# KTH-RPL/HiMo

Hardware: AMD Instinct MI355X
Metric: lidar_frames_per_sec_120k (higher is better)
Workload: dtype f16x2 (two-term split fp16, x = h + l with exact subnormals, on the matrix cores; float32 accumulate; ~22-bit products); 1 GPU; per-frame pipeline: pillarise 3 sweeps (512x512 grid) -> SeFlow++-style encoder/decoder + GRU head (random-init, self-specified: reference network source absent) -> per-point flow -> ego-motion removal + dt0 + flow2compDis -> comp_dis; points_per_frame=120000, sweeps_per_frame=3, parallelism=frames sharded x1, refined_output=False, batches_in_flight=3, matrix_arithmetic=f16x2, samples_per_backbone_launch=16, collectives=none (single process)

## Files before the change

### himo_amd/csrc/gruhead.hip

```cpp
#include "conv_common.h"
#include "bf16x3.h"

namespace himo {

struct GruHeadArgs {
    int64_t n;
    const int* pid; const float* offsets;
    const float* img0; const float* img1; int img_pitch;
    const float* dec; int dec_pitch;
    const float* w_off; const float* b_off;
    const unsigned short* wzr; const float* bzr;
    const unsigned short* wq; const float* bq;
    const unsigned short* w1; const float* b1;
    const float* w2; const float* b2;
    const float* xyz_t; const float* pts; int stride;
    float* flow;
    int iters;
    int img_split;
    unsigned* nonfinite;
    int w2_pitch;
};

constexpr int kGhMaxIters = 4;
struct GruHeadSave {
    float* hx;
    float* rhx;
    float* z; float* r; float* q;
    float* pre1; float* y1;
    float* res;
    int64_t rows;
};

constexpr int kGhMaxSamples = 16;
struct GruHeadSample {
    int64_t n;
    const int* pid; const float* offsets; const float* img0; const float* img1; const float* dec;
    const float* xyz_t; const float* pts; float* flow; int stride;
};
struct GruHeadBatch {
    int n_samples;
    int block_start[kGhMaxSamples + 1];
    GruHeadSample s[kGhMaxSamples];
};

constexpr int kGhRows = 64;
constexpr bool kGhLaunder = false;

template <int SLABS>
__device__ inline int a_slot(int s, int slab, int row, int half) {
    return ((s * SLABS + slab) * kGhRows + row) * 32 + ((half ^ ((row >> 4) & 1)) << 4);
}

template <int FMT, int SLABS>
__device__ inline void a_store(unsigned char* A, int row, int k, float v) {
    constexpr int kGhPlane = SLABS * kGhRows * 32;
    unsigned h, m = 0, l;
    if (FMT == 3) split3(v, h, m, l); else split2(v, h, l);
    const int slab = k >> 4, kk = k & 15;
    const int off = a_slot<SLABS>(0, slab, row, kk >> 3) + (kk & 7) * 2;
    *reinterpret_cast<unsigned short*>(A + off) = (unsigned short)h;
    if (FMT == 3) *reinterpret_cast<unsigned short*>(A + off + kGhPlane) = (unsigned short)m;
    *reinterpret_cast<unsigned short*>(A + off + (FMT - 1) * kGhPlane) = (unsigned short)l;
}

template <int RT, int NT, int FMT, int SLABS>
__device__ inline void gemm192(const unsigned char* A, const unsigned short* __restrict__ wpk, int cout, const int (&col)[NT],
                               floatx16 (&acc)[RT][NT], int rt0, int li, int lh) {
    uint4 bcur[NT][FMT], bnxt[NT][FMT];
    auto load_b = [&](int slab, uint4 (&b)[NT][FMT]) {
#pragma unroll
        for (int t = 0; t < NT; ++t)
#pragma unroll
            for (int s = 0; s < FMT; ++s)
                b[t][s] = *reinterpret_cast<const uint4*>(wpk + (((int64_t)slab * FMT + s) * cout + col[t] + li) * 16 + lh * 8);
    };
    load_b(0, bcur);
    constexpr int kUnroll = SLABS % 2 == 0 ? 2 : 3;
#pragma unroll kUnroll
    for (int slab = 0; slab < SLABS; ++slab) {
        if (slab + 1 < SLABS) load_b(slab + 1, bnxt);
        bf16x8 af[RT][FMT];
#pragma unroll
        for (int rt = 0; rt < RT; ++rt)
#pragma unroll
            for (int s = 0; s < FMT; ++s)
                af[rt][s] = *reinterpret_cast<const bf16x8*>(A + a_slot<SLABS>(s, slab, (rt0 + rt) * 32 + li, lh));
#define HIMO_TERM(SA, SB)                                                                                          \
    _Pragma("unroll") for (int rt = 0; rt < RT; ++rt) _Pragma("unroll") for (int t = 0; t < NT; ++t)                  \
        acc[rt][t] = __builtin_amdgcn_mfma_f32_32x32x16_bf16(af[rt][SA], __builtin_bit_cast(bf16x8, bcur[t][SB]), acc[rt][t], 0, 0, 0);
#define HIMO_TERM16(ACC, SA, SB)                                                                                   \
    _Pragma("unroll") for (int rt = 0; rt < RT; ++rt) _Pragma("unroll") for (int t = 0; t < NT; ++t)                  \
        ACC[rt][t] = __builtin_amdgcn_mfma_f32_32x32x16_f16(__builtin_bit_cast(f16x8, af[rt][SA]),                    \
                                                           __builtin_bit_cast(f16x8, bcur[t][SB]), ACC[rt][t], 0, 0, 0);
        if constexpr (FMT == 3) {
            HIMO_TERM(2, 0) HIMO_TERM(0, 2) HIMO_TERM(1, 1) HIMO_TERM(1, 0) HIMO_TERM(0, 1) HIMO_TERM(0, 0)
        } else {
            HIMO_TERM16(acc, 1, 0) HIMO_TERM16(acc, 0, 1) HIMO_TERM16(acc, 0, 0)
        }
#undef HIMO_TERM16
#undef HIMO_TERM
#pragma unroll
        for (int t = 0; t < NT; ++t)
#pragma unroll
            for (int s = 0; s < FMT; ++s) bcur[t][s] = bnxt[t][s];
    }
    if (FMT == 2) {
#pragma unroll
        for (int rt = 0; rt < RT; ++rt)
#pragma unroll
            for (int t = 0; t < NT; ++t)
#pragma unroll
                for (int r = 0; r < 16; ++r)
                    acc[rt][t][r] = acc[rt][t][r] * kF16AccScale;
    }
}

template <int GROUP>
__device__ inline void sv_store(float* base, unsigned byte_off, float v) {
    *reinterpret_cast<float*>(reinterpret_cast<char*>(base) + byte_off) = v;
}

template <int FMT, int SLABS, bool SAVE = false>
__global__ __launch_bounds__(256, (FMT == 2 && !SAVE) ? 3 : 2) void gru_head_kernel(GruHeadArgs a, GruHeadBatch batch, GruHeadSave sv) {
    constexpr bool FOLD = SLABS == 9;
    static_assert(!(SAVE && FOLD), "the training forward keeps x explicit");
    constexpr int kGhPlane = SLABS * kGhRows * 32;
    __shared__ __attribute__((aligned(16))) unsigned char A[FMT * kGhPlane];
    __shared__ int s_pid[kGhRows];
    const int wave = __builtin_amdgcn_readfirstlane(threadIdx.x >> 6), lane = threadIdx.x & 63;
    const int li = lane & 31, lh = lane >> 5;
    int bid = blockIdx.x;
    {
        int smp = 0;
        while (smp + 1 < batch.n_samples && bid >= batch.block_start[smp + 1]) ++smp;
        bid -= batch.block_start[smp];
        const GruHeadSample& g = batch.s[smp];
        a.n = g.n; a.pid = g.pid; a.offsets = g.offsets; a.img0 = g.img0; a.img1 = g.img1; a.dec = g.dec;
        a.xyz_t = g.xyz_t; a.pts = g.pts; a.flow = g.flow; a.stride = g.stride;
    }
    const int64_t r0 = (int64_t)bid * kGhRows;

    if (threadIdx.x < kGhRows) {
        const int64_t i = r0 + threadIdx.x;
        s_pid[threadIdx.x] = i < a.n ? a.pid[i] : -1;
    }
    if constexpr (FOLD) {
        const int row = threadIdx.x >> 2, q = threadIdx.x & 3;
        const int64_t i = r0 + row;
        float v[4] = {0.f, 0.f, 0.f, 0.f};
        if (q == 0) {
            if (i < a.n) { v[0] = a.offsets[i * 3]; v[1] = a.offsets[i * 3 + 1]; v[2] = a.offsets[i * 3 + 2]; }
            v[3] = 1.f;
        }
#pragma unroll
        for (int k = 0; k < 4; ++k) a_store<FMT, SLABS>(A, row, 128 + q * 4 + k, v[k]);
    } else if constexpr (SAVE) {
        const int c = threadIdx.x & 63;
        const float w0 = a.w_off[c], w1 = a.w_off[64 + c], w2 = a.w_off[128 + c], bc = a.b_off[c];
#pragma unroll 4
        for (int j = 0; j < 16; ++j) {
            const int row = wave + 4 * j;
            const int64_t i = r0 + row;
            const int64_t ic = i < a.n ? i : a.n - 1;
            const float o0 = a.offsets[ic * 3], o1 = a.offsets[ic * 3 + 1], o2 = a.offsets[ic * 3 + 2];
            const float v = fmaf(o2, w2, fmaf(o1, w1, o0 * w0)) + bc;
            a_store<FMT, SLABS>(A, row, 128 + c, v);
            const unsigned at = ((unsigned)i * 192u + 128u + (unsigned)c) * 4u;
            for (int t = 0; t <= a.iters; ++t) sv_store<0>(sv.hx + t * sv.rows * 192, at, v);
            for (int t = 0; t < a.iters; ++t) sv_store<0>(sv.rhx + t * sv.rows * 192, at, v);
        }
    } else {
        const int row = threadIdx.x >> 2, q = threadIdx.x & 3;
        const int64_t i = r0 + row;
        float o0 = 0.f, o1 = 0.f, o2 = 0.f;
        if (i < a.n) { o0 = a.offsets[i * 3]; o1 = a.offsets[i * 3 + 1]; o2 = a.offsets[i * 3 + 2]; }
#pragma unroll
        for (int k = 0; k < 16; ++k) {
            const int c = q * 16 + k;
            const float v = fmaf(o2, a.w_off[128 + c], fmaf(o1, a.w_off[64 + c], o0 * a.w_off[c])) + a.b_off[c];
            a_store<FMT, SLABS>(A, row, 128 + c, v);
        }
    }
    __syncthreads();

    const float* src = wave == 0 ? a.img0 : wave == 1 ? a.img1 : a.dec + (wave - 2) * 32;
    const int src_pitch = wave < 2 ? a.img_pitch : a.dec_pitch;
    float h[2][16];
    {
        int cell[2][16];
#pragma unroll
        for (int rt = 0; rt < 2; ++rt)
#pragma unroll
            for (int r = 0; r < 16; ++r) cell[rt][r] = s_pid[rt * 32 + (r & 3) + 8 * (r >> 2) + 4 * lh];
        if (FMT == 2 && wave < 2 && a.img_split) {
            unsigned short hh[2][16], ll[2][16];
#pragma unroll
            for (int rt = 0; rt < 2; ++rt)
#pragma unroll
                for (int r = 0; r < 16; ++r) {
                    const unsigned short* rec = reinterpret_cast<const unsigned short*>(src + (int64_t)max(cell[rt][r], 0) * src_pitch + (li & ~15));
                    hh[rt][r] = rec[li & 15]; ll[rt][r] = rec[16 + (li & 15)];
                }
#pragma unroll
            for (int rt = 0; rt < 2; ++rt)
#pragma unroll
                for (int r = 0; r < 16; ++r)
                    h[rt][r] = cell[rt][r] >= 0 ? (float)__builtin_bit_cast(_Float16, hh[rt][r]) + (float)__builtin_bit_cast(_Float16, ll[rt][r]) : 0.f;
        } else {
#pragma unroll
            for (int rt = 0; rt < 2; ++rt)
#pragma unroll
                for (int r = 0; r < 16; ++r) h[rt][r] = src[(int64_t)max(cell[rt][r], 0) * src_pitch + li];
#pragma unroll
            for (int rt = 0; rt < 2; ++rt)
#pragma unroll
                for (int r = 0; r < 16; ++r) h[rt][r] = cell[rt][r] >= 0 ? h[rt][r] : 0.f;
            if (FMT == 2 && wave < 2) {
#pragma unroll
                for (int rt = 0; rt < 2; ++rt)
#pragma unroll
                    for (int r = 0; r < 16; ++r) {
                        unsigned hh, ll;
                        split2(h[rt][r], hh, ll);
                        h[rt][r] = (float)__builtin_bit_cast(_Float16, (unsigned short)hh) + (float)__builtin_bit_cast(_Float16, (unsigned short)ll);
                    }
            }
        }
#pragma unroll
        for (int rt = 0; rt < 2; ++rt)
#pragma unroll
            for (int r = 0; r < 16; ++r) {
                const int row = rt * 32 + (r & 3) + 8 * (r >> 2) + 4 * lh;
                a_store<FMT, SLABS>(A, row, wave * 32 + li, h[rt][r]);
                if constexpr (SAVE) sv_store<1>(sv.hx, (((unsigned)r0 + row) * 192u + wave * 32 + li) * 4u, h[rt][r]);
            }
    }
    __syncthreads();
    unsigned o128 = (((unsigned)r0 + 4 * lh) * 128u + wave * 32 + li) * 4u, o192 = (((unsigned)r0 + 4 * lh) * 192u + wave * 32 + li) * 4u;

    const int col_zr[2] = {wave * 32, 128 + wave * 32};
    const int col_q[1] = {wave * 32};
    const float bz = a.bzr[wave * 32 + li], br = a.bzr[128 + wave * 32 + li], bq = a.bq[wave * 32 + li];

#pragma unroll 1
    for (int it = 0; it < a.iters; ++it) {
        int sli = li, slh = lh;
        if constexpr (SAVE || kGhLaunder) asm volatile("" : "+v"(o128), "+v"(o192), "+v"(sli), "+v"(slh));
        float* const sz = SAVE ? sv.z + it * sv.rows * 128 : nullptr; float* const sr = SAVE ? sv.r + it * sv.rows * 128 : nullptr;
        float* const sq = SAVE ? sv.q + it * sv.rows * 128 : nullptr; float* const srhx = SAVE ? sv.rhx + it * sv.rows * 192 : nullptr;
        float* const shx = SAVE ? sv.hx + (it + 1) * sv.rows * 192 : nullptr;
        floatx16 acc[2][2];
#pragma unroll
        for (int rt = 0; rt < 2; ++rt)
#pragma unroll
            for (int t = 0; t < 2; ++t)
#pragma unroll
                for (int r = 0; r < 16; ++r) acc[rt][t][r] = 0.f;
        gemm192<2, 2, FMT, SLABS>(A, a.wzr, 256, col_zr, acc, 0, li, lh);
        __syncthreads();
#pragma unroll
        for (int rt = 0; rt < 2; ++rt)
#pragma unroll
            for (int r = 0; r < 16; ++r) {
                acc[rt][0][r] = sigmoid_f(acc[rt][0][r] + bz);
                const float rr = sigmoid_f(acc[rt][1][r] + br);
                const int row = rt * 32 + (r & 3) + 8 * (r >> 2) + 4 * slh;
                a_store<FMT, SLABS>(A, row, wave * 32 + sli, rr * h[rt][r]);
                if constexpr (SAVE) {
                    const unsigned dr = rt * 32 + (r & 3) + 8 * (r >> 2);
                    sv_store<2>(sz, o128 + dr * 512u, acc[rt][0][r]); sv_store<2>(sr, o128 + dr * 512u, rr);
                    sv_store<3>(srhx, o192 + dr * 768u, rr * h[rt][r]);
                }
            }
        __syncthreads();
        if constexpr (SAVE || kGhLaunder) asm volatile("" : "+v"(o128), "+v"(o192), "+v"(sli), "+v"(slh));
        floatx16 acq[2][1];
#pragma unroll
        for (int rt = 0; rt < 2; ++rt)
#pragma unroll
            for (int r = 0; r < 16; ++r) acq[rt][0][r] = 0.f;
        gemm192<2, 1, FMT, SLABS>(A, a.wq, 128, col_q, acq, 0, li, lh);
        __syncthreads();
#pragma unroll
        for (int rt = 0; rt < 2; ++rt)
#pragma unroll
            for (int r = 0; r < 16; ++r) {
                const float q = tanh_f(acq[rt][0][r] + bq);
                const float zz = acc[rt][0][r];
                const float hn = (1.0f - zz) * h[rt][r] + zz * q;
                h[rt][r] = hn;
                const int row = rt * 32 + (r & 3) + 8 * (r >> 2) + 4 * slh;
                a_store<FMT, SLABS>(A, row, wave * 32 + sli, hn);
                if constexpr (SAVE) {
                    const unsigned dr = rt * 32 + (r & 3) + 8 * (r >> 2);
                    sv_store<4>(sq, o128 + dr * 512u, q);
                    sv_store<5>(shx, o192 + dr * 768u, hn);
                }
            }
        __syncthreads();
    }

    floatx16 ac1[1][1];
#pragma unroll
    for (int r = 0; r < 16; ++r) ac1[0][0][r] = 0.f;
    const int col_1[1] = {0};
    if (wave < 2) gemm192<1, 1, FMT, SLABS>(A, a.w1, 32, col_1, ac1, wave, li, lh);
    __syncthreads();
    float* Y = reinterpret_cast<float*>(A);
    if (wave < 2) {
        const float b1 = a.b1[li];
#pragma unroll
        for (int r = 0; r < 16; ++r) {
            const int row = wave * 32 + (r & 3) + 8 * (r >> 2) + 4 * lh;
            const float pre = ac1[0][0][r] + b1, y = gelu_exact(pre);
            Y[row * 32 + li] = y;
            if constexpr (SAVE) {
                const unsigned at = (((unsigned)r0 + row) * 32u + li) * 4u;
                sv_store<6>(sv.pre1, at, pre); sv_store<6>(sv.y1, at, y);
            }
        }
    }
    __syncthreads();
    if constexpr (SAVE) {
        const int row = threadIdx.x >> 2, c = threadIdx.x & 3;
        const int64_t i = r0 + row;
        float out = 0.f;
        if (c < 3 && s_pid[row] >= 0) {
            const float* y = Y + row * 32;
            float s = y[0] * a.w2[c];
#pragma unroll
            for (int k = 1; k < 32; ++k) s = fmaf(y[k], a.w2[k * a.w2_pitch + c], s);
            out = s + a.b2[c];
        }
        sv.res[i * 4 + c] = out;
        if (a.nonfinite && !(fabsf(out) <= 3.4028234664e38f)) atomicOr(a.nonfinite, 1u);
        return;
    }
    if (threadIdx.x < 3 * kGhRows) {
        const int row = threadIdx.x / 3, c = threadIdx.x % 3;
        const int64_t i = r0 + row;
        if (i < a.n) {
            const float pose_flow = a.xyz_t[i * 3 + c] - a.pts[i * a.stride + c];
            float out = pose_flow;
            if (s_pid[row] >= 0) {
                const float* y = Y + row * 32;
                float s = y[0] * a.w2[c];
#pragma unroll
                for (int k = 1; k < 32; ++k) s = fmaf(y[k], a.w2[k * a.w2_pitch + c], s);
                out = pose_flow + (s + a.b2[c]);
            }
            a.flow[i * 3 + c] = out;
            if (a.nonfinite && !(fabsf(out) <= 3.4028234664e38f)) atomicOr(a.nonfinite, 1u);
        }
    }
}

}

using namespace himo;

static int gru_head_launch(int n_samples, const himo_head_sample* h_samples, int img_pitch, int dec_pitch,
                           const float* d_w_off, const float* d_b_off, bool folded,
                           const void* d_wzr_packed, const float* d_bzr, const void* d_wq_packed, const float* d_bq,
                           const void* d_w1_packed, const float* d_b1, const float* d_w2, const float* d_b2,
                           int iters, int packed_format, int img_split, unsigned* d_nonfinite, void* stream) {
    if (img_split && (packed_format != 1 || (img_pitch & 15))) return HIMO_ERR_INVALID_ARGUMENT;
    if (n_samples < 0 || n_samples > kGhMaxSamples || (n_samples && !h_samples)) return HIMO_ERR_INVALID_ARGUMENT;
    if (iters < 0 || !(packed_format == 0 || packed_format == 1) || img_pitch < 32 || dec_pitch < 64) return HIMO_ERR_INVALID_ARGUMENT;
    if ((!folded && (!d_w_off || !d_b_off)) || !d_wzr_packed || !d_bzr || !d_wq_packed || !d_bq || !d_w1_packed || !d_b1 || !d_w2 || !d_b2)
        return HIMO_ERR_INVALID_ARGUMENT;
    if ((reinterpret_cast<uintptr_t>(d_wzr_packed) | reinterpret_cast<uintptr_t>(d_wq_packed) | reinterpret_cast<uintptr_t>(d_w1_packed)) & 15)
        return HIMO_ERR_INVALID_ARGUMENT;
    GruHeadBatch b{};
    int64_t blocks = 0;
    for (int i = 0; i < n_samples; ++i) {
        const himo_head_sample& h = h_samples[i];
        if (h.n < 0 || h.pc_stride < 3) return HIMO_ERR_INVALID_ARGUMENT;
        if (h.n == 0) continue;
        if (!h.d_pid || !h.d_offsets || !h.d_img0 || !h.d_img1 || !h.d_dec || !h.d_xyz_t || !h.d_pts || !h.d_flow) return HIMO_ERR_INVALID_ARGUMENT;
        GruHeadSample& g = b.s[b.n_samples];
        g.n = h.n; g.pid = h.d_pid; g.offsets = h.d_offsets; g.img0 = h.d_img0; g.img1 = h.d_img1; g.dec = h.d_dec;
        g.xyz_t = h.d_xyz_t; g.pts = h.d_pts; g.flow = h.d_flow; g.stride = h.pc_stride;
        b.block_start[b.n_samples] = (int)blocks;
        blocks += (h.n + kGhRows - 1) / kGhRows;
        if (blocks > 0x7fffffff) return HIMO_ERR_INVALID_ARGUMENT;
        b.block_start[++b.n_samples] = (int)blocks;
    }
    if (!blocks) return HIMO_OK;
    GruHeadArgs a{};
    a.img_pitch = img_pitch; a.dec_pitch = dec_pitch; a.w_off = d_w_off; a.b_off = d_b_off;
    a.wzr = (const unsigned short*)d_wzr_packed; a.bzr = d_bzr; a.wq = (const unsigned short*)d_wq_packed; a.bq = d_bq;
    a.w1 = (const unsigned short*)d_w1_packed; a.b1 = d_b1; a.w2 = d_w2; a.b2 = d_b2; a.iters = iters;
    a.img_split = img_split ? 1 : 0;
    a.nonfinite = d_nonfinite;
    a.w2_pitch = 3;
    hipStream_t s = (hipStream_t)stream;
    ProfScope ps("gru_head_kernel", s);
    const dim3 grid((unsigned)blocks);
    const GruHeadSave none{};
    if (folded) {
        if (packed_format == 1) hipLaunchKernelGGL((gru_head_kernel<2, 9>), grid, dim3(256), 0, s, a, b, none);
        else hipLaunchKernelGGL((gru_head_kernel<3, 9>), grid, dim3(256), 0, s, a, b, none);
    } else {
        if (packed_format == 1) hipLaunchKernelGGL((gru_head_kernel<2, 12>), grid, dim3(256), 0, s, a, b, none);
        else hipLaunchKernelGGL((gru_head_kernel<3, 12>), grid, dim3(256), 0, s, a, b, none);
    }
    HIMO_LAUNCH_CHECK("gru_head_kernel");
    return HIMO_OK;
}

extern "C" int himo_gru_head_batch(int n_samples, const himo_head_sample* h_samples, int img_pitch, int dec_pitch,
                                   const float* d_w_off, const float* d_b_off,
                                   const void* d_wzr_packed, const float* d_bzr, const void* d_wq_packed, const float* d_bq,
                                   const void* d_w1_packed, const float* d_b1, const float* d_w2, const float* d_b2,
                                   int iters, int packed_format, int img_split, void* stream) {
    return gru_head_launch(n_samples, h_samples, img_pitch, dec_pitch, d_w_off, d_b_off, false, d_wzr_packed, d_bzr, d_wq_packed, d_bq,
                           d_w1_packed, d_b1, d_w2, d_b2, iters, packed_format, img_split, nullptr, stream);
}

extern "C" int himo_gru_head_batch_folded(int n_samples, const himo_head_sample* h_samples, int img_pitch, int dec_pitch,
                                          const void* d_wzr_packed, const float* d_bzr, const void* d_wq_packed, const float* d_bq,
                                          const void* d_w1_packed, const float* d_b1, const float* d_w2, const float* d_b2,
                                          int iters, int packed_format, int img_split, void* stream) {
    return gru_head_launch(n_samples, h_samples, img_pitch, dec_pitch, nullptr, nullptr, true, d_wzr_packed, d_bzr, d_wq_packed, d_bq,
                           d_w1_packed, d_b1, d_w2, d_b2, iters, packed_format, img_split, nullptr, stream);
}

extern "C" int himo_gru_head_batch_guarded(int n_samples, const himo_head_sample* h_samples, int img_pitch, int dec_pitch,
                                           const float* d_w_off, const float* d_b_off,
                                           const void* d_wzr_packed, const float* d_bzr, const void* d_wq_packed, const float* d_bq,
                                           const void* d_w1_packed, const float* d_b1, const float* d_w2, const float* d_b2,
                                           int iters, int packed_format, int img_split, uint32_t* d_nonfinite, void* stream) {
    if ((d_w_off == nullptr) != (d_b_off == nullptr)) return HIMO_ERR_INVALID_ARGUMENT;
    return gru_head_launch(n_samples, h_samples, img_pitch, dec_pitch, d_w_off, d_b_off, d_w_off == nullptr, d_wzr_packed, d_bzr, d_wq_packed,
                           d_bq, d_w1_packed, d_b1, d_w2, d_b2, iters, packed_format, img_split, d_nonfinite, stream);
}

extern "C" int himo_gru_head_train(int64_t n, const int32_t* d_pid, const float* d_offsets, const float* d_img0, const float* d_img1,
                                   int img_pitch, const float* d_dec, int dec_pitch, const float* d_w_off, const float* d_b_off,
                                   const void* d_wzr_packed, const float* d_bzr, const void* d_wq_packed, const float* d_bq,
                                   const void* d_w1_packed, const float* d_b1, const float* d_w2, int w2_pitch, const float* d_b2,
                                   int iters, int packed_format, const himo_head_saved* h_saved, uint32_t* d_nonfinite, void* stream) {
    if (n < 0 || iters < 1 || iters > kGhMaxIters || !(packed_format == 0 || packed_format == 1) || img_pitch < 32 || dec_pitch < 64 ||
        !(w2_pitch == 3 || w2_pitch == 4) || !h_saved)
        return HIMO_ERR_INVALID_ARGUMENT;
    if (!d_w_off || !d_b_off || !d_wzr_packed || !d_bzr || !d_wq_packed || !d_bq || !d_w1_packed || !d_b1 || !d_w2 || !d_b2)
        return HIMO_ERR_INVALID_ARGUMENT;
    if ((reinterpret_cast<uintptr_t>(d_wzr_packed) | reinterpret_cast<uintptr_t>(d_wq_packed) | reinterpret_cast<uintptr_t>(d_w1_packed)) & 15)
        return HIMO_ERR_INVALID_ARGUMENT;
    if (n == 0) return HIMO_OK;
    if (!d_pid || !d_offsets || !d_img0 || !d_img1 || !d_dec) return HIMO_ERR_INVALID_ARGUMENT;
    if (h_saved && h_saved->rows * 768 >= ((int64_t)1 << 32)) return HIMO_ERR_UNSUPPORTED;
    GruHeadSave sv{};
    sv.hx = h_saved->d_hx; sv.rhx = h_saved->d_rhx; sv.z = h_saved->d_z; sv.r = h_saved->d_r; sv.q = h_saved->d_q;
    sv.pre1 = h_saved->d_pre1; sv.y1 = h_saved->d_y1; sv.res = h_saved->d_res;
    sv.rows = h_saved->rows;
    if (!sv.hx || !sv.rhx || !sv.z || !sv.r || !sv.q || !sv.pre1 || !sv.y1 || !sv.res || sv.rows < (n + 63) / 64 * 64 || (sv.rows & 63))
        return HIMO_ERR_INVALID_ARGUMENT;
    GruHeadBatch b{};
    b.n_samples = 1;
    GruHeadSample& g = b.s[0];
    g.n = n; g.pid = d_pid; g.offsets = d_offsets; g.img0 = d_img0; g.img1 = d_img1; g.dec = d_dec;
    const int64_t blocks = (n + kGhRows - 1) / kGhRows;
    if (blocks > 0x7fffffff) return HIMO_ERR_INVALID_ARGUMENT;
    b.block_start[0] = 0; b.block_start[1] = (int)blocks;
    GruHeadArgs a{};
    a.img_pitch = img_pitch; a.dec_pitch = dec_pitch; a.w_off = d_w_off; a.b_off = d_b_off;
    a.wzr = (const unsigned short*)d_wzr_packed; a.bzr = d_bzr; a.wq = (const unsigned short*)d_wq_packed; a.bq = d_bq;
    a.w1 = (const unsigned short*)d_w1_packed; a.b1 = d_b1; a.w2 = d_w2; a.b2 = d_b2; a.iters = iters; a.w2_pitch = w2_pitch;
    a.nonfinite = d_nonfinite;
    hipStream_t s = (hipStream_t)stream;
    ProfScope ps("gru_head_train_kernel", s);
    if (packed_format == 1) hipLaunchKernelGGL((gru_head_kernel<2, 12, true>), dim3((unsigned)blocks), dim3(256), 0, s, a, b, sv);
    else hipLaunchKernelGGL((gru_head_kernel<3, 12, true>), dim3((unsigned)blocks), dim3(256), 0, s, a, b, sv);
    HIMO_LAUNCH_CHECK("gru_head_kernel<train>");
    return HIMO_OK;
}

extern "C" int himo_clear_u32(uint32_t* d_words, int n, void* stream) {
    if (!d_words || n < 1) return HIMO_ERR_INVALID_ARGUMENT;
    HIMO_HIP(hipMemsetAsync(d_words, 0, (size_t)n * 4, (hipStream_t)stream));
    return HIMO_OK;
}

extern "C" int himo_gru_head(int64_t n, const int32_t* d_pid, const float* d_offsets, const float* d_img0, const float* d_img1,
                             int img_pitch, const float* d_dec, int dec_pitch, const float* d_w_off, const float* d_b_off,
                             const void* d_wzr_packed, const float* d_bzr, const void* d_wq_packed, const float* d_bq,
                             const void* d_w1_packed, const float* d_b1, const float* d_w2, const float* d_b2,
                             const float* d_xyz_t, const float* d_pts, int pc_stride, float* d_flow, int iters, int packed_format,
                             void* stream) {
    himo_head_sample h{n, d_pid, d_offsets, d_img0, d_img1, d_dec, d_xyz_t, d_pts, pc_stride, d_flow};
    return himo_gru_head_batch(1, &h, img_pitch, dec_pitch, d_w_off, d_b_off, d_wzr_packed, d_bzr, d_wq_packed, d_bq,
                               d_w1_packed, d_b1, d_w2, d_b2, iters, packed_format, 0, stream);
}
```

Baseline: 757.6 frames/s.

## Widen folded f16x2 GRU head blocks to 128 rows with buffer-load double-buffered weights

The folded f16x2 GRU head now processes 128 rows per 256-thread block, so each wave handles four row tiles and every weight fragment loaded from global memory feeds twice as many MFMAs. The weight loads switch to raw buffer loads through a buffer resource, and the slab loop is restructured into an explicit two-buffer ping-pong that computes one row tile at a time. Separately, the r*h product and the GRU blend are computed with contraction disabled, and the product is split into two fp16 terms via an fma residual. The trade-off is twice the LDS per block and a lower occupancy target (2 blocks instead of 3), plus higher register pressure from the larger accumulator arrays.

```diff
diff --git a/himo_amd/csrc/gruhead.hip b/himo_amd/csrc/gruhead.hip
--- a/himo_amd/csrc/gruhead.hip
+++ b/himo_amd/csrc/gruhead.hip
@@ -44,65 +44,104 @@
 };
 
 constexpr int kGhRows = 64;
+constexpr int kGhRowsWide = 128;
 constexpr bool kGhLaunder = false;
 
-template <int SLABS>
+template <int SLABS, int ROWS>
 __device__ inline int a_slot(int s, int slab, int row, int half) {
-    return ((s * SLABS + slab) * kGhRows + row) * 32 + ((half ^ ((row >> 4) & 1)) << 4);
-}
-
-template <int FMT, int SLABS>
+    return ((s * SLABS + slab) * ROWS + row) * 32 + ((half ^ ((row >> 4) & 1)) << 4);
+}
+
+template <int FMT, int SLABS, int ROWS>
 __device__ inline void a_store(unsigned char* A, int row, int k, float v) {
-    constexpr int kGhPlane = SLABS * kGhRows * 32;
+    constexpr int kGhPlane = SLABS * ROWS * 32;
     unsigned h, m = 0, l;
     if (FMT == 3) split3(v, h, m, l); else split2(v, h, l);
     const int slab = k >> 4, kk = k & 15;
-    const int off = a_slot<SLABS>(0, slab, row, kk >> 3) + (kk & 7) * 2;
+    const int off = a_slot<SLABS, ROWS>(0, slab, row, kk >> 3) + (kk & 7) * 2;
     *reinterpret_cast<unsigned short*>(A + off) = (unsigned short)h;
     if (FMT == 3) *reinterpret_cast<unsigned short*>(A + off + kGhPlane) = (unsigned short)m;
     *reinterpret_cast<unsigned short*>(A + off + (FMT - 1) * kGhPlane) = (unsigned short)l;
 }
 
-template <int RT, int NT, int FMT, int SLABS>
+template <int FMT, int SLABS, int ROWS>
+__device__ inline void a_store_prod(unsigned char* A, int row, int k, float r, float h) {
+    if constexpr (FMT == 2) {
+#pragma clang fp contract(off)
+        const _Float16 hh = (_Float16)(r * h);
+        const _Float16 ll = (_Float16)fmaf(r, h, -(float)hh);
+        const int slab = k >> 4, kk = k & 15;
+        const int off = a_slot<SLABS, ROWS>(0, slab, row, kk >> 3) + (kk & 7) * 2;
+        *reinterpret_cast<unsigned short*>(A + off) = __builtin_bit_cast(unsigned short, hh);
+        *reinterpret_cast<unsigned short*>(A + off + SLABS * ROWS * 32) = __builtin_bit_cast(unsigned short, ll);
+    } else {
+        a_store<FMT, SLABS, ROWS>(A, row, k, r * h);
+    }
+}
+template <int FMT>
+__device__ inline float gru_blend(float z, float h, float q) {
+    if constexpr (FMT == 2) {
+#pragma clang fp contract(off)
+        const float a = (1.0f - z) * h, b = z * q;
+        return a + b;
+    } else {
+        return (1.0f - z) * h + z * q;
+    }
+}
+
+template <int RT, int NT, int FMT, int SLABS, int ROWS>
 __device__ inline void gemm192(const unsigned char* A, const unsigned short* __restrict__ wpk, int cout, const int (&col)[NT],
                                floatx16 (&acc)[RT][NT], int rt0, int li, int lh) {
-    uint4 bcur[NT][FMT], bnxt[NT][FMT];
+    uint4 b0[NT][FMT], b1[NT][FMT];
+    const __amdgpu_buffer_rsrc_t wrsrc = __builtin_amdgcn_make_buffer_rsrc(const_cast<unsigned short*>(wpk), 0, SLABS * FMT * cout * 32, 0x00020000);
+    const int lane_off = li * 32 + lh * 16;
     auto load_b = [&](int slab, uint4 (&b)[NT][FMT]) {
+        typedef unsigned u32x4 __attribute__((ext_vector_type(4)));
 #pragma unroll
         for (int t = 0; t < NT; ++t)
 #pragma unroll
+            for (int s = 0; s < FMT; ++s) {
+                const u32x4 v = __builtin_amdgcn_raw_buffer_load_b128(wrsrc, lane_off, ((slab * FMT + s) * cout + col[t]) * 32, 0);
+                b[t][s] = __builtin_bit_cast(uint4, v);
+            }
+    };
+    auto step = [&](int slab, const uint4 (&b)[NT][FMT]) {
+#pragma unroll
+        for (int rt = 0; rt < RT; ++rt) {
+            bf16x8 af[FMT];
+#pragma unroll
             for (int s = 0; s < FMT; ++s)
-                b[t][s] = *reinterpret_cast<const uint4*>(wpk + (((int64_t)slab * FMT + s) * cout + col[t] + li) * 16 + lh * 8);
-    };
-    load_b(0, bcur);
-    constexpr int kUnroll = SLABS % 2 == 0 ? 2 : 3;
-#pragma unroll kUnroll
-    for (int slab = 0; slab < SLABS; ++slab) {
-        if (slab + 1 < SLABS) load_b(slab + 1, bnxt);
-        bf16x8 af[RT][FMT];
-#pragma unroll
-        for (int rt = 0; rt < RT; ++rt)
-#pragma unroll
-            for (int s = 0; s < FMT; ++s)
-                af[rt][s] = *reinterpret_cast<const bf16x8*>(A + a_slot<SLABS>(s, slab, (rt0 + rt) * 32 + li, lh));
+                af[s] = *reinterpret_cast<const bf16x8*>(A + a_slot<SLABS, ROWS>(s, slab, (rt0 + rt) * 32 + li, lh));
 #define HIMO_TERM(SA, SB)                                                                                          \
-    _Pragma("unroll") for (int rt = 0; rt < RT; ++rt) _Pragma("unroll") for (int t = 0; t < NT; ++t)                  \
-        acc[rt][t] = __builtin_amdgcn_mfma_f32_32x32x16_bf16(af[rt][SA], __builtin_bit_cast(bf16x8, bcur[t][SB]), acc[rt][t], 0, 0, 0);
-#define HIMO_TERM16(ACC, SA, SB)                                                                                   \
-    _Pragma("unroll") for (int rt = 0; rt < RT; ++rt) _Pragma("unroll") for (int t = 0; t < NT; ++t)                  \
-        ACC[rt][t] = __builtin_amdgcn_mfma_f32_32x32x16_f16(__builtin_bit_cast(f16x8, af[rt][SA]),                    \
-                                                           __builtin_bit_cast(f16x8, bcur[t][SB]), ACC[rt][t], 0, 0, 0);
-        if constexpr (FMT == 3) {
-            HIMO_TERM(2, 0) HIMO_TERM(0, 2) HIMO_TERM(1, 1) HIMO_TERM(1, 0) HIMO_TERM(0, 1) HIMO_TERM(0, 0)
-        } else {
-            HIMO_TERM16(acc, 1, 0) HIMO_TERM16(acc, 0, 1) HIMO_TERM16(acc, 0, 0)
-        }
+    _Pragma("unroll") for (int t = 0; t < NT; ++t)                                                                    \
+        acc[rt][t] = __builtin_amdgcn_mfma_f32_32x32x16_bf16(af[SA], __builtin_bit_cast(bf16x8, b[t][SB]), acc[rt][t], 0, 0, 0);
+#define HIMO_TERM16(SA, SB)                                                                                        \
+    _Pragma("unroll") for (int t = 0; t < NT; ++t)                                                                    \
+        acc[rt][t] = __builtin_amdgcn_mfma_f32_32x32x16_f16(__builtin_bit_cast(f16x8, af[SA]),                        \
+                                                           __builtin_bit_cast(f16x8, b[t][SB]), acc[rt][t], 0, 0, 0);
+            if constexpr (FMT == 3) {
+                HIMO_TERM(2, 0) HIMO_TERM(0, 2) HIMO_TERM(1, 1) HIMO_TERM(1, 0) HIMO_TERM(0, 1) HIMO_TERM(0, 0)
+            } else {
+                HIMO_TERM16(1, 0) HIMO_TERM16(0, 1) HIMO_TERM16(0, 0)
+            }
 #undef HIMO_TERM16
 #undef HIMO_TERM
-#pragma unroll
-        for (int t = 0; t < NT; ++t)
-#pragma unroll
-            for (int s = 0; s < FMT; ++s) bcur[t][s] = bnxt[t][s];
+        }
+    };
+    load_b(0, b0);
+#pragma unroll 1
+    for (int slab = 0; slab + 2 < SLABS; slab += 2) {
+        load_b(slab + 1, b1);
+        step(slab, b0);
+        load_b(slab + 2, b0);
+        step(slab + 1, b1);
+    }
+    if constexpr (SLABS % 2 == 1) {
+        step(SLABS - 1, b0);
+    } else {
+        load_b(SLABS - 1, b1);
+        step(SLABS - 2, b0);
+        step(SLABS - 1, b1);
     }
     if (FMT == 2) {
 #pragma unroll
@@ -120,13 +159,16 @@
     *reinterpret_cast<float*>(reinterpret_cast<char*>(base) + byte_off) = v;
 }
 
-template <int FMT, int SLABS, bool SAVE = false>
-__global__ __launch_bounds__(256, (FMT == 2 && !SAVE) ? 3 : 2) void gru_head_kernel(GruHeadArgs a, GruHeadBatch batch, GruHeadSave sv) {
+template <int FMT, int SLABS, bool SAVE = false, int ROWS = kGhRows>
+__global__ __launch_bounds__(256, (FMT == 2 && !SAVE && ROWS == 64) ? 3 : 2) void gru_head_kernel(GruHeadArgs a, GruHeadBatch batch, GruHeadSave sv) {
     constexpr bool FOLD = SLABS == 9;
+    constexpr int RT = ROWS / 32;
     static_assert(!(SAVE && FOLD), "the training forward keeps x explicit");
-    constexpr int kGhPlane = SLABS * kGhRows * 32;
+    static_assert(ROWS == 64 || ROWS == 128, "a wave owns 32 hidden columns of 2 or 4 row tiles");
+    static_assert(!SAVE || ROWS == kGhRows, "the saved tensors are laid out for 64-row blocks");
+    constexpr int kGhPlane = SLABS * ROWS * 32;
     __shared__ __attribute__((aligned(16))) unsigned char A[FMT * kGhPlane];
-    __shared__ int s_pid[kGhRows];
+    __shared__ int s_pid[ROWS];
     const int wave = __builtin_amdgcn_readfirstlane(threadIdx.x >> 6), lane = threadIdx.x & 63;
     const int li = lane & 31, lh = lane >> 5;
     int bid = blockIdx.x;
@@ -138,22 +180,25 @@
         a.n = g.n; a.pid = g.pid; a.offsets = g.offsets; a.img0 = g.img0; a.img1 = g.img1; a.dec = g.dec;
         a.xyz_t = g.xyz_t; a.pts = g.pts; a.flow = g.flow; a.stride = g.stride;
     }
-    const int64_t r0 = (int64_t)bid * kGhRows;
-
-    if (threadIdx.x < kGhRows) {
+    const int64_t r0 = (int64_t)bid * ROWS;
+
+    if (threadIdx.x < ROWS) {
         const int64_t i = r0 + threadIdx.x;
         s_pid[threadIdx.x] = i < a.n ? a.pid[i] : -1;
     }
     if constexpr (FOLD) {
-        const int row = threadIdx.x >> 2, q = threadIdx.x & 3;
-        const int64_t i = r0 + row;
-        float v[4] = {0.f, 0.f, 0.f, 0.f};
-        if (q == 0) {
-            if (i < a.n) { v[0] = a.offsets[i * 3]; v[1] = a.offsets[i * 3 + 1]; v[2] = a.offsets[i * 3 + 2]; }
-            v[3] = 1.f;
-        }
-#pragma unroll
-        for (int k = 0; k < 4; ++k) a_store<FMT, SLABS>(A, row, 128 + q * 4 + k, v[k]);
+#pragma unroll
+        for (int rb = 0; rb < ROWS; rb += 64) {
+            const int row = rb + (threadIdx.x >> 2), q = threadIdx.x & 3;
+            const int64_t i = r0 + row;
+            float v[4] = {0.f, 0.f, 0.f, 0.f};
+            if (q == 0) {
+                if (i < a.n) { v[0] = a.offsets[i * 3]; v[1] = a.offsets[i * 3 + 1]; v[2] = a.offsets[i * 3 + 2]; }
+                v[3] = 1.f;
+            }
+#pragma unroll
+            for (int k = 0; k < 4; ++k) a_store<FMT, SLABS, ROWS>(A, row, 128 + q * 4 + k, v[k]);
+        }
     } else if constexpr (SAVE) {
         const int c = threadIdx.x & 63;
         const float w0 = a.w_off[c], w1 = a.w_off[64 + c], w2 = a.w_off[128 + c], bc = a.b_off[c];
@@ -164,76 +209,80 @@
             const int64_t ic = i < a.n ? i : a.n - 1;
             const float o0 = a.offsets[ic * 3], o1 = a.offsets[ic * 3 + 1], o2 = a.offsets[ic * 3 + 2];
             const float v = fmaf(o2, w2, fmaf(o1, w1, o0 * w0)) + bc;
-            a_store<FMT, SLABS>(A, row, 128 + c, v);
+            a_store<FMT, SLABS, ROWS>(A, row, 128 + c, v);
             const unsigned at = ((unsigned)i * 192u + 128u + (unsigned)c) * 4u;
             for (int t = 0; t <= a.iters; ++t) sv_store<0>(sv.hx + t * sv.rows * 192, at, v);
             for (int t = 0; t < a.iters; ++t) sv_store<0>(sv.rhx + t * sv.rows * 192, at, v);
         }
     } else {
-        const int row = threadIdx.x >> 2, q = threadIdx.x & 3;
-        const int64_t i = r0 + row;
-        float o0 = 0.f, o1 = 0.f, o2 = 0.f;
-        if (i < a.n) { o0 = a.offsets[i * 3]; o1 = a.offsets[i * 3 + 1]; o2 = a.offsets[i * 3 + 2]; }
-#pragma unroll
-        for (int k = 0; k < 16; ++k) {
-            const int c = q * 16 + k;
-            const float v = fmaf(o2, a.w_off[128 + c], fmaf(o1, a.w_off[64 + c], o0 * a.w_off[c])) + a.b_off[c];
-            a_store<FMT, SLABS>(A, row, 128 + c, v);
+#pragma unroll
+        for (int rb = 0; rb < ROWS; rb += 64) {
+            const int row = rb + (threadIdx.x >> 2), q = threadIdx.x & 3;
+            const int64_t i = r0 + row;
+            float o0 = 0.f, o1 = 0.f, o2 = 0.f;
+            if (i < a.n) { o0 = a.offsets[i * 3]; o1 = a.offsets[i * 3 + 1]; o2 = a.offsets[i * 3 + 2]; }
+#pragma unroll
+            for (int k = 0; k < 16; ++k) {
+                const int c = q * 16 + k;
+                const float v = fmaf(o2, a.w_off[128 + c], fmaf(o1, a.w_off[64 + c], o0 * a.w_off[c])) + a.b_off[c];
+                a_store<FMT, SLABS, ROWS>(A, row, 128 + c, v);
+            }
         }
     }
     __syncthreads();
 
     const float* src = wave == 0 ? a.img0 : wave == 1 ? a.img1 : a.dec + (wave - 2) * 32;
     const int src_pitch = wave < 2 ? a.img_pitch : a.dec_pitch;
-    float h[2][16];
-    {
-        int cell[2][16];
-#pragma unroll
-        for (int rt = 0; rt < 2; ++rt)
-#pragma unroll
-            for (int r = 0; r < 16; ++r) cell[rt][r] = s_pid[rt * 32 + (r & 3) + 8 * (r >> 2) + 4 * lh];
-        if (FMT == 2 && wave < 2 && a.img_split) {
-            unsigned short hh[2][16], ll[2][16];
+    float h[RT][16];
+#pragma unroll
+    for (int rp = 0; rp < RT; rp += 2) {
+            int cell[2][16];
 #pragma unroll
             for (int rt = 0; rt < 2; ++rt)
 #pragma unroll
+                for (int r = 0; r < 16; ++r) cell[rt][r] = s_pid[(rp + rt) * 32 + (r & 3) + 8 * (r >> 2) + 4 * lh];
+            if (FMT == 2 && wave < 2 && a.img_split) {
+                unsigned short hh[2][16], ll[2][16];
+#pragma unroll
+                for (int rt = 0; rt < 2; ++rt)
+#pragma unroll
+                    for (int r = 0; r < 16; ++r) {
+                        const unsigned short* rec = reinterpret_cast<const unsigned short*>(src + (int64_t)max(cell[rt][r], 0) * src_pitch + (li & ~15));
+                        hh[rt][r] = rec[li & 15]; ll[rt][r] = rec[16 + (li & 15)];
+                    }
+#pragma unroll
+                for (int rt = 0; rt < 2; ++rt)
+#pragma unroll
+                    for (int r = 0; r < 16; ++r)
+                        h[rp + rt][r] = cell[rt][r] >= 0 ? (float)__builtin_bit_cast(_Float16, hh[rt][r]) + (float)__builtin_bit_cast(_Float16, ll[rt][r]) : 0.f;
+            } else {
+#pragma unroll
+                for (int rt = 0; rt < 2; ++rt)
+#pragma unroll
+                    for (int r = 0; r < 16; ++r) h[rp + rt][r] = src[(int64_t)max(cell[rt][r], 0) * src_pitch + li];
+#pragma unroll
+                for (int rt = 0; rt < 2; ++rt)
+#pragma unroll
+                    for (int r = 0; r < 16; ++r) h[rp + rt][r] = cell[rt][r] >= 0 ? h[rp + rt][r] : 0.f;
+                if (FMT == 2 && wave < 2) {
+#pragma unroll
+                    for (int rt = 0; rt < 2; ++rt)
+#pragma unroll
+                        for (int r = 0; r < 16; ++r) {
+                            unsigned hh, ll;
+                            split2(h[rp + rt][r], hh, ll);
+                            h[rp + rt][r] = (float)__builtin_bit_cast(_Float16, (unsigned short)hh) + (float)__builtin_bit_cast(_Float16, (unsigned short)ll);
+                        }
+                }
+            }
+#pragma unroll
+            for (int rt = 0; rt < 2; ++rt)
+#pragma unroll
                 for (int r = 0; r < 16; ++r) {
-                    const unsigned short* rec = reinterpret_cast<const unsigned short*>(src + (int64_t)max(cell[rt][r], 0) * src_pitch + (li & ~15));
-                    hh[rt][r] = rec[li & 15]; ll[rt][r] = rec[16 + (li & 15)];
+                    const int row = (rp + rt) * 32 + (r & 3) + 8 * (r >> 2) + 4 * lh;
+                    a_store<FMT, SLABS, ROWS>(A, row, wave * 32 + li, h[rp + rt][r]);
+                    if constexpr (SAVE) sv_store<1>(sv.hx, (((unsigned)r0 + row) * 192u + wave * 32 + li) * 4u, h[rp + rt][r]);
                 }
-#pragma unroll
-            for (int rt = 0; rt < 2; ++rt)
-#pragma unroll
-                for (int r = 0; r < 16; ++r)
-                    h[rt][r] = cell[rt][r] >= 0 ? (float)__builtin_bit_cast(_Float16, hh[rt][r]) + (float)__builtin_bit_cast(_Float16, ll[rt][r]) : 0.f;
-        } else {
-#pragma unroll
-            for (int rt = 0; rt < 2; ++rt)
-#pragma unroll
-                for (int r = 0; r < 16; ++r) h[rt][r] = src[(int64_t)max(cell[rt][r], 0) * src_pitch + li];
-#pragma unroll
-            for (int rt = 0; rt < 2; ++rt)
-#pragma unroll
-                for (int r = 0; r < 16; ++r) h[rt][r] = cell[rt][r] >= 0 ? h[rt][r] : 0.f;
-            if (FMT == 2 && wave < 2) {
-#pragma unroll
-                for (int rt = 0; rt < 2; ++rt)
-#pragma unroll
-                    for (int r = 0; r < 16; ++r) {
-                        unsigned hh, ll;
-                        split2(h[rt][r], hh, ll);
-                        h[rt][r] = (float)__builtin_bit_cast(_Float16, (unsigned short)hh) + (float)__builtin_bit_cast(_Float16, (unsigned short)ll);
-                    }
-            }
-        }
-#pragma unroll
-        for (int rt = 0; rt < 2; ++rt)
-#pragma unroll
-            for (int r = 0; r < 16; ++r) {
-                const int row = rt * 32 + (r & 3) + 8 * (r >> 2) + 4 * lh;
-                a_store<FMT, SLABS>(A, row, wave * 32 + li, h[rt][r]);
-                if constexpr (SAVE) sv_store<1>(sv.hx, (((unsigned)r0 + row) * 192u + wave * 32 + li) * 4u, h[rt][r]);
-            }
     }
     __syncthreads();
     unsigned o128 = (((unsigned)r0 + 4 * lh) * 128u + wave * 32 + li) * 4u, o192 = (((unsigned)r0 + 4 * lh) * 192u + wave * 32 + li) * 4u;
@@ -249,23 +298,23 @@
         float* const sz = SAVE ? sv.z + it * sv.rows * 128 : nullptr; float* const sr = SAVE ? sv.r + it * sv.rows * 128 : nullptr;
         float* const sq = SAVE ? sv.q + it * sv.rows * 128 : nullptr; float* const srhx = SAVE ? sv.rhx + it * sv.rows * 192 : nullptr;
         float* const shx = SAVE ? sv.hx + (it + 1) * sv.rows * 192 : nullptr;
-        floatx16 acc[2][2];
-#pragma unroll
-        for (int rt = 0; rt < 2; ++rt)
+        floatx16 acc[RT][2];
+#pragma unroll
+        for (int rt = 0; rt < RT; ++rt)
 #pragma unroll
             for (int t = 0; t < 2; ++t)
 #pragma unroll
                 for (int r = 0; r < 16; ++r) acc[rt][t][r] = 0.f;
-        gemm192<2, 2, FMT, SLABS>(A, a.wzr, 256, col_zr, acc, 0, li, lh);
+        gemm192<RT, 2, FMT, SLABS, ROWS>(A, a.wzr, 256, col_zr, acc, 0, li, lh);
         __syncthreads();
 #pragma unroll
-        for (int rt = 0; rt < 2; ++rt)
+        for (int rt = 0; rt < RT; ++rt)
 #pragma unroll
             for (int r = 0; r < 16; ++r) {
                 acc[rt][0][r] = sigmoid_f(acc[rt][0][r] + bz);
                 const float rr = sigmoid_f(acc[rt][1][r] + br);
                 const int row = rt * 32 + (r & 3) + 8 * (r >> 2) + 4 * slh;
-                a_store<FMT, SLABS>(A, row, wave * 32 + sli, rr * h[rt][r]);
+                a_store_prod<FMT, SLABS, ROWS>(A, row, wave * 32 + sli, rr, h[rt][r]);
                 if constexpr (SAVE) {
                     const unsigned dr = rt * 32 + (r & 3) + 8 * (r >> 2);
                     sv_store<2>(sz, o128 + dr * 512u, acc[rt][0][r]); sv_store<2>(sr, o128 + dr * 512u, rr);
@@ -274,23 +323,23 @@
             }
         __syncthreads();
         if constexpr (SAVE || kGhLaunder) asm volatile("" : "+v"(o128), "+v"(o192), "+v"(sli), "+v"(slh));
-        floatx16 acq[2][1];
-#pragma unroll
-        for (int rt = 0; rt < 2; ++rt)
+        floatx16 acq[RT][1];
+#pragma unroll
+        for (int rt = 0; rt < RT; ++rt)
 #pragma unroll
             for (int r = 0; r < 16; ++r) acq[rt][0][r] = 0.f;
-        gemm192<2, 1, FMT, SLABS>(A, a.wq, 128, col_q, acq, 0, li, lh);
+        gemm192<RT, 1, FMT, SLABS, ROWS>(A, a.wq, 128, col_q, acq, 0, li, lh);
         __syncthreads();
 #pragma unroll
-        for (int rt = 0; rt < 2; ++rt)
+        for (int rt = 0; rt < RT; ++rt)
 #pragma unroll
             for (int r = 0; r < 16; ++r) {
                 const float q = tanh_f(acq[rt][0][r] + bq);
                 const float zz = acc[rt][0][r];
-                const float hn = (1.0f - zz) * h[rt][r] + zz * q;
+                const float hn = gru_blend<FMT>(zz, h[rt][r], q);
                 h[rt][r] = hn;
                 const int row = rt * 32 + (r & 3) + 8 * (r >> 2) + 4 * slh;
-                a_store<FMT, SLABS>(A, row, wave * 32 + sli, hn);
+                a_store<FMT, SLABS, ROWS>(A, row, wave * 32 + sli, hn);
                 if constexpr (SAVE) {
                     const unsigned dr = rt * 32 + (r & 3) + 8 * (r >> 2);
                     sv_store<4>(sq, o128 + dr * 512u, q);
@@ -304,10 +353,10 @@
 #pragma unroll
     for (int r = 0; r < 16; ++r) ac1[0][0][r] = 0.f;
     const int col_1[1] = {0};
-    if (wave < 2) gemm192<1, 1, FMT, SLABS>(A, a.w1, 32, col_1, ac1, wave, li, lh);
+    if (wave < RT) gemm192<1, 1, FMT, SLABS, ROWS>(A, a.w1, 32, col_1, ac1, wave, li, lh);
     __syncthreads();
     float* Y = reinterpret_cast<float*>(A);
-    if (wave < 2) {
+    if (wave < RT) {
         const float b1 = a.b1[li];
 #pragma unroll
         for (int r = 0; r < 16; ++r) {
@@ -336,8 +385,8 @@
         if (a.nonfinite && !(fabsf(out) <= 3.4028234664e38f)) atomicOr(a.nonfinite, 1u);
         return;
     }
-    if (threadIdx.x < 3 * kGhRows) {
-        const int row = threadIdx.x / 3, c = threadIdx.x % 3;
+    for (int e = threadIdx.x; e < 3 * ROWS; e += 256) {
+        const int row = e / 3, c = e % 3;
         const int64_t i = r0 + row;
         if (i < a.n) {
             const float pose_flow = a.xyz_t[i * 3 + c] - a.pts[i * a.stride + c];
@@ -371,6 +420,7 @@
         return HIMO_ERR_INVALID_ARGUMENT;
     if ((reinterpret_cast<uintptr_t>(d_wzr_packed) | reinterpret_cast<uintptr_t>(d_wq_packed) | reinterpret_cast<uintptr_t>(d_w1_packed)) & 15)
         return HIMO_ERR_INVALID_ARGUMENT;
+    const int rows = (folded && packed_format == 1) ? kGhRowsWide : kGhRows;
     GruHeadBatch b{};
     int64_t blocks = 0;
     for (int i = 0; i < n_samples; ++i) {
@@ -382,7 +432,7 @@
         g.n = h.n; g.pid = h.d_pid; g.offsets = h.d_offsets; g.img0 = h.d_img0; g.img1 = h.d_img1; g.dec = h.d_dec;
         g.xyz_t = h.d_xyz_t; g.pts = h.d_pts; g.flow = h.d_flow; g.stride = h.pc_stride;
         b.block_start[b.n_samples] = (int)blocks;
-        blocks += (h.n + kGhRows - 1) / kGhRows;
+        blocks += (h.n + rows - 1) / rows;
         if (blocks > 0x7fffffff) return HIMO_ERR_INVALID_ARGUMENT;
         b.block_start[++b.n_samples] = (int)blocks;
     }
@@ -399,7 +449,7 @@
     const dim3 grid((unsigned)blocks);
     const GruHeadSave none{};
     if (folded) {
-        if (packed_format == 1) hipLaunchKernelGGL((gru_head_kernel<2, 9>), grid, dim3(256), 0, s, a, b, none);
+        if (packed_format == 1) hipLaunchKernelGGL((gru_head_kernel<2, 9, false, kGhRowsWide>), grid, dim3(256), 0, s, a, b, none);
         else hipLaunchKernelGGL((gru_head_kernel<3, 9>), grid, dim3(256), 0, s, a, b, none);
     } else {
         if (packed_format == 1) hipLaunchKernelGGL((gru_head_kernel<2, 12>), grid, dim3(256), 0, s, a, b, none);
```

Result: no change. 754.7 frames/s (-0.4%).
